# tobwei/APTAI

Hardware: AMD Instinct MI355X
Metric: utterances/sec (10 s @ 16 kHz) train-step (higher is better)
Workload: dtype bf16

## Files before the change

aptai_amd/_lib.py:

```python
from __future__ import annotations

import ctypes
import os
import subprocess
import threading

import torch

_HERE = os.path.dirname(os.path.abspath(__file__))
CSRC = os.path.join(_HERE, "csrc")
LIB_PATH = os.environ.get("APTAI_HIP_LIB") or os.path.join(CSRC, "libaptai_hip.so")

_lib = None
_lock = threading.Lock()

_P, _I64, _I, _F, _U64 = ctypes.c_void_p, ctypes.c_int64, ctypes.c_int, ctypes.c_float, ctypes.c_uint64
ARGTYPES = {
    "aptai_layernorm_fwd": [_P, _P, _P, _P, _P, _P, _I64, _I64, _F, _I, _P],
    "aptai_layernorm_bwd": [_P, _P, _P, _P, _P, _P, _P, _P, _F, _U64, _P, _P, _P, _I64, _I64, _P, _P],
    "aptai_layernorm_bwd_workspace_bytes": [_I64, _I64],
    "aptai_layernorm_bwd_finalize_multi": [_P, _I64, _I64, _P],
    "aptai_layernorm_fwd_f32in": [_P, _P, _P, _P, _P, _I64, _I64, _F, _P],
    "aptai_layernorm_fwd_f32in_split": [_P, _P, _P, _P, _P, _I, _I64, _I64, _F, _P],
    "aptai_attention_fwd": [_P, _P, _P, _P, _P, _I64, _I64, _I64, _I64, _F, _F, _U64, _I, _P],
    "aptai_attention_bwd": [_P, _P, _P, _P, _P, _P, _P, _P, _I64, _I64, _I64, _I64, _F, _F, _U64, _I, _I, _P],
    "aptai_cast_f32_to_bf16": [_P, _P, _I64, _I64, _I64, _P],
    "aptai_conv_weight_to_bf16": [_P, _P, _I64, _I64, _I64, _P],
    "aptai_posconv_weight": [_P, _P, _P, _P, _P, _I64, _I64, _I64, _P],
    "aptai_posconv_pack": [_P, _P, _P, _P, _I64, _I64, _I64, _I64, _I64, _P],
    "aptai_frame_mask_fwd": [_P, _P, _P, _P, _I64, _I64, _I64, _I64, _P],
    "aptai_frame_mask_bwd": [_P, _P, _P, _P, _P, _I64, _I64, _I64, _I64, _P],
    "aptai_frame_mask_bwd_workspace_bytes": [_I64, _I64, _I64],
    "aptai_colsum_bf16": [_P, _I64, _P, _P, _I64, _I64, _I, _P],
    "aptai_colsum_workspace_bytes": [_I64, _I64],
    "aptai_dropout_bf16": [_P, _P, _I64, _F, _U64, _P],
    "aptai_dgelu_bf16": [_P, _P, _P, _I64, _P],
    "aptai_conv0_fwd": [_P, _I64, _I64, _P, _P, _P, _P, _I, _F, _P, _I64, _I64, _I64, _I64, _I64, _P, _P, _P],
    "aptai_conv0_bwd": [_P, _I64, _I64, _P, _P, _P, _P, _I, _F, _P, _I64, _I64, _P, _P, _P, _P, _P, _P, _P],
    "aptai_conv0_bwd_workspace_bytes": [_I64, _I64],
    "aptai_conv0_bwd_data": [_P, _I64, _I64, _P, _P, _P, _P, _I, _F, _P, _I64, _I64, _P, _P, _P, _P],
    "aptai_conv0_bwd_data_workspace_bytes": [_I64, _I64],
    "aptai_conv0_workspace_bytes": [_I64, _I64],
    "aptai_head_act_fwd": [_P, _P, _P, _I64, _F, _F, _U64, _P],
    "aptai_head_act_bwd": [_P, _P, _P, _P, _I64, _F, _F, _U64, _P],
    "aptai_lowpass_fir": [_P, _I64, _I64, _P, _I64, _P, _I64, _I64, _I, _I64, _I64, _I64, _I64, _I64, _P],
    "aptai_aptai_loss_fwd": [_P, _P, _P, _I64, _I64, _P, _I64, _I64, _I64, _I64, _F, _F, _P, _P, _P, _P],
    "aptai_aptai_loss_bwd": [_P, _P, _P, _I64, _I64, _P, _I64, _I64, _I64, _I64, _F, _F, _P, _P, _P, _P, _I64, _P],
    "aptai_aptai_loss_workspace_bytes": [],
# ... 97 lines not shown
```

aptai_amd/csrc/attention.hip:

```cpp
#include "common.h"

namespace {

#ifdef APTAI_STAMPS
__device__ unsigned long long g_attn_stamps[3 * 1024 * 8];
#define ATTN_STAMP(k, slot)                                                                                       \
    do {                                                                                                          \
        if (threadIdx.x == 0) {                                                                                   \
            const int bl = blockIdx.x + gridDim.x * (blockIdx.y + gridDim.y * blockIdx.z);                        \
            if (bl < 1024) g_attn_stamps[((k) * 1024 + bl) * 8 + (slot)] = wall_clock64();                         \
        }                                                                                                         \
    } while (0)
#else
#define ATTN_STAMP(k, slot) do {} while (0)
#endif

constexpr int HD = 64;
constexpr float LOG2E = 1.4426950408889634f;

struct AttnArgs {
    const bf16_t* qkv; long ld;
    const int* lens;
    bf16_t* ctx; long ldo;
    float* lse2;
    float* o32;
    int B, Tp, H, heads;
    float c;
    float scale;
    uint32_t seed0, seed1, thr16; float dscale;
    const uint32_t* salt;
    const bf16_t* dctx;
    float* delta;
    bf16_t* dqkv;
    int skip_pad_q;
    int stagger;
    int xcd_remap;
// ... 54 lines not shown
    const int r31 = lane & 31, h = lane >> 5;
#pragma unroll
    for (int dt = 0; dt < 2; ++dt)
#pragma unroll
        for (int g4 = 0; g4 < 4; ++g4) {
            const int d = dt * 32 + 8 * g4 + 4 * h;
            *(u32x2*)(sw + r31 * OUT_PITCH + d * 2) = (u32x2){pack2bf(acc[dt][4 * g4] * scale, acc[dt][4 * g4 + 1] * scale),
                                                              pack2bf(acc[dt][4 * g4 + 2] * scale, acc[dt][4 * g4 + 3] * scale)};
        }
    __builtin_amdgcn_fence(__ATOMIC_RELEASE, "wavefront");
#pragma unroll
    for (int i = 0; i < 4; ++i) {
        const int idx = i * 64 + lane, r = idx >> 3, ch = idx & 7;
        *(u32x4*)(g_row0 + (long)r * ld + ch * 8) = *(const u32x4*)(sw + r * OUT_PITCH + ch * 16);
    }
    __builtin_amdgcn_fence(__ATOMIC_ACQUIRE, "wavefront");
}

__device__ __forceinline__ bool attn_keep(uint32_t pair, int key, uint32_t s0, uint32_t s1, uint32_t thr16) {
    const uint32_t hsh = rng_hash(pair, s0, s1);
    return ((key & 1) ? (hsh >> 16) : (hsh & 0xffffu)) >= thr16;
}

__device__ __forceinline__ void attn_block(const AttnArgs& a, int& tile, int& hd, int& b) {
    const int nt = gridDim.x, total = nt * gridDim.y * gridDim.z;
    int L = blockIdx.x + nt * (blockIdx.y + gridDim.y * blockIdx.z);
    if (a.xcd_remap && (total & 7) == 0) L = (L & 7) * (total >> 3) + (L >> 3);
    tile = L % nt;
    const int grp = L / nt;
    hd = grp % (int)gridDim.y;
    b = grp / (int)gridDim.y;
}

constexpr int FWD_BUF = 2 * 64 * 128;
constexpr int FWD_SMEM = 2 * FWD_BUF;
constexpr float REF_HEADROOM = 40.0f;
constexpr float REF_SUM_LIMIT = 1.4901161193847656e-08f;

template <bool V> struct Flag { static constexpr bool value = V; };

template <bool DROP>
__global__ __launch_bounds__(256, 3) void attn_fwd_kernel(AttnArgs a) {
    __shared__ __attribute__((aligned(16))) char smem[FWD_SMEM];
    ATTN_STAMP(0, 0);
    if (DROP) apply_salt(a.salt, a.seed0, a.seed1);
    const int tid = threadIdx.x, lane = tid & 63, wave = tid >> 6, h = lane >> 5;
    int tile_x, hd, b;
    attn_block(a, tile_x, hd, b);
    const int q0 = tile_x * 128 + wave * 32;
    int len = a.lens[b];
    len = len < 1 ? 1 : (len > a.Tp ? a.Tp : len);
    const int ntiles = (len + 63) >> 6;
    const long rowbase = (long)b * a.Tp;
    const int q = q0 + (lane & 31);
    const bf16_t* Qg = a.qkv + (rowbase + q) * a.ld + hd * HD;
// ... 153 lines not shown
    if (a.o32) {
#pragma unroll
        for (int dt = 0; dt < 2; ++dt) {
            __syncthreads();
#pragma unroll
            for (int g4 = 0; g4 < 4; ++g4)
                *(f32x4*)(sw + r31 * OUT_PITCH + (8 * g4 + 4 * h) * 4) =
                    (f32x4){oT[dt][4 * g4], oT[dt][4 * g4 + 1], oT[dt][4 * g4 + 2], oT[dt][4 * g4 + 3]};
            __syncthreads();
#pragma unroll
            for (int i = 0; i < 4; ++i) {
                const int idx = i * 64 + lane, r = idx >> 3, ch = idx & 7;
                *(f32x4*)(a.o32 + orow + (long)r * a.ldo + dt * 32 + ch * 4) = *(const f32x4*)(sw + r * OUT_PITCH + ch * 16);
            }
        }
    }
    ATTN_STAMP(0, 3);
#ifdef APTAI_STAMPS
    asm volatile("s_waitcnt vmcnt(0)" ::: "memory");
    ATTN_STAMP(0, 4);
#endif
}

template <bool PRE>
__global__ __launch_bounds__(256, PRE ? DKDV_BLOCKS : 2) void attn_bwd_dkdv_kernel(AttnArgs a) {
    __shared__ __attribute__((aligned(16))) char smem[STAGE_BYTES + 384 + DKDV_KV_BYTES];
    char* sQ = smem;
    char* sD = smem + 32 * 128;
    float* sL = (float*)(smem + STAGE_BYTES);
    char* sKall = smem + STAGE_BYTES + 384;
    char* sVall = sKall + 128 * 128;
    ATTN_STAMP(1, 0);
    if (a.thr16) apply_salt(a.salt, a.seed0, a.seed1);
    const int tid = threadIdx.x, lane = tid & 63, wave = tid >> 6, h = lane >> 5;
    int tile_x, hd, b;
    attn_block(a, tile_x, hd, b);
    const int kb0 = tile_x * 128;
    const int key0 = kb0 + wave * 32;
    int len = a.lens[b];
    len = len < 1 ? 1 : (len > a.Tp ? a.Tp : len);
    const long rowbase = (long)b * a.Tp;
    const int key = key0 + (lane & 31);
    bf16_t* dK0 = a.dqkv + (rowbase + kb0) * a.ld + a.H + hd * HD;
    bf16_t* dV0 = dK0 + a.H;
    if (kb0 >= len) {
        const u32x4 z = {0u, 0u, 0u, 0u};
#pragma unroll
        for (int it = 0; it < 4; ++it) {
            const int cid = it * 256 + tid, row = cid >> 3, ch = cid & 7;
            *(u32x4*)(dK0 + (long)row * a.ld + ch * 8) = z;
            *(u32x4*)(dV0 + (long)row * a.ld + ch * 8) = z;
        }
        return;
    }
    const LaneOffs lo = lane_offs(lane);
    const bf16_t* K0 = a.qkv + (rowbase + kb0) * a.ld + a.H + hd * HD;
    stage_rows128(sKall, K0, a.ld, tid);
    stage_rows128(sVall, K0 + a.H, a.ld, tid);
    f32x16 dKT[2], dVT[2];
    dKT[0] = dKT[1] = dVT[0] = dVT[1] = (f32x16)(0.f);

    const int nq = a.skip_pad_q ? ((len + 31) >> 5) : (a.Tp >> 5);
    const bf16_t* Qb = a.qkv + rowbase * a.ld + hd * HD;
    const bf16_t* Db = a.dctx + rowbase * a.ldo + hd * HD;
    const float* lse = a.lse2 + ((long)b * a.heads + hd) * a.Tp;
    const float* del = a.delta + ((long)b * a.heads + hd) * a.Tp;
    const int srow = tid >> 3, sch = tid & 7;
    const int soff = tile_off(srow, sch);
    const long gq = (long)srow * a.ld + sch * 8, gd = (long)srow * a.ldo + sch * 8;
    u32x4 qreg = *(const u32x4*)(Qb + gq), dreg = *(const u32x4*)(Db + gd);
    const float* stat = (tid < 8 ? lse : del) + (tid & 7) * 4;
    f32x4 sreg = (f32x4)(0.f);
    if (tid < 16) sreg = *(const f32x4*)stat;
    const bool key_ok = key < len;
    const bool wave_boundary = key0 + 32 > len;
    const uint32_t hshift = (key & 1) ? 16u : 0u;
    const float c = a.c;
    const uint32_t pairk = (uint32_t)(key >> 1) * ATTN_K1;
    const uint32_t rowid0 = (uint32_t)((b * a.heads + hd) * a.Tp) + (uint32_t)(tid & 31);
    uint32_t hreg = 0;
    if (a.thr16 && tid >= 32 && tid < 64) hreg = rng_hash(rowid0, a.seed0, a.seed1);
    ATTN_STAMP(1, 1);
    for (int t = 0; t < nq; ++t) {
        __syncthreads();
        *(u32x4*)(sQ + soff) = qreg;
        *(u32x4*)(sD + soff) = dreg;
        if (tid < 16) *(f32x4*)(sL + tid * 4) = PRE ? -sreg : sreg;
        if (a.thr16 && tid >= 32 && tid < 64) ((uint32_t*)sL)[64 + (tid & 31)] = hreg;
        __syncthreads();
        if (t + 1 < nq) {
            qreg = *(const u32x4*)(Qb + (long)(t + 1) * 32 * a.ld + gq);
            dreg = *(const u32x4*)(Db + (long)(t + 1) * 32 * a.ldo + gd);
            if (tid < 16) sreg = *(const f32x4*)(stat + (t + 1) * 32);
            if (a.thr16 && tid >= 32 && tid < 64) hreg = rng_hash(rowid0 + (uint32_t)((t + 1) * 32), a.seed0, a.seed1);
        }
        f32x16 cs = (f32x16)(0.f), cd = (f32x16)(0.f);
        if (PRE) {
#pragma unroll
            for (int g4 = 0; g4 < 4; ++g4) {
                const f32x4 l4 = *(const f32x4*)(sL + 8 * g4 + 4 * h);
                const f32x4 d4 = *(const f32x4*)(sL + 32 + 8 * g4 + 4 * h);
#pragma unroll
                for (int rr = 0; rr < 4; ++rr) { cs[4 * g4 + rr] = l4[rr]; cd[4 * g4 + rr] = d4[rr]; }
            }
        }
        f32x16 s = __builtin_amdgcn_mfma_f32_32x32x16_bf16(rd_row(sQ, lo, 0, 0), rd_row(sKall, lo, wave, 0), cs, 0, 0, 0);
        f32x16 dp = __builtin_amdgcn_mfma_f32_32x32x16_bf16(rd_row(sD, lo, 0, 0), rd_row(sVall, lo, wave, 0), cd, 0, 0, 0);
#pragma unroll
        for (int ds = 1; ds < 4; ++ds) {
            s = __builtin_amdgcn_mfma_f32_32x32x16_bf16(rd_row(sQ, lo, 0, ds), rd_row(sKall, lo, wave, ds), s, 0, 0, 0);
            dp = __builtin_amdgcn_mfma_f32_32x32x16_bf16(rd_row(sD, lo, 0, ds), rd_row(sVall, lo, wave, ds), dp, 0, 0, 0);
        }
        float pd[16], dsv[16];
        if (PRE) {
#pragma unroll
            for (int r = 0; r < 16; ++r) pd[r] = fast_exp2(s[r]);
// ... 26 lines not shown
                    const bool k = ((y >> hshift) & 0xffffu) >= a.thr16;
                    const float p0 = pd[r];
                    if (PRE) dsv[r] = p0 * (k ? dp[r] : nd4[rr]);
                    else dsv[r] = p0 * ((k ? dp[r] : 0.f) - dsv[r]);
                    pd[r] = k ? p0 : 0.f;
                }
            }
        } else {
#pragma unroll
            for (int r = 0; r < 16; ++r) dsv[r] = PRE ? pd[r] * dp[r] : pd[r] * (dp[r] - dsv[r]);
        }
#pragma unroll
        for (int sstep = 0; sstep < 2; ++sstep) {
            const bf16x8 pf = pack8(&pd[8 * sstep]);
            const bf16x8 df = pack8(&dsv[8 * sstep]);
#pragma unroll
            for (int dt = 0; dt < 2; ++dt) {
                dVT[dt] = __builtin_amdgcn_mfma_f32_32x32x16_bf16(rd_tr(sD, lo, sstep, dt), pf, dVT[dt], 0, 0, 0);
                dKT[dt] = __builtin_amdgcn_mfma_f32_32x32x16_bf16(rd_tr(sQ, lo, sstep, dt), df, dKT[dt], 0, 0, 0);
            }
        }
    }
    __syncthreads();
    ATTN_STAMP(1, 2);
    char* sw = smem + wave * (32 * OUT_PITCH);
    store_rows_bf16(sw, dKT, (PRE ? 0.6931471805599453f : a.scale) * a.dscale, dK0 + (long)(wave * 32) * a.ld, a.ld, lane);
    store_rows_bf16(sw, dVT, a.dscale, dV0 + (long)(wave * 32) * a.ld, a.ld, lane);
    ATTN_STAMP(1, 3);
#ifdef APTAI_STAMPS
    asm volatile("s_waitcnt vmcnt(0)" ::: "memory");
    ATTN_STAMP(1, 4);
#endif
}

template <bool PRE>
__global__ __launch_bounds__(256, 3) void attn_bwd_dq_kernel(AttnArgs a) {
    __shared__ __attribute__((aligned(16))) char smem[DQ_STAGE + 512];
    char* sK = smem;
    char* sV = smem + 32 * 128;
    float* sDel = (float*)(smem + DQ_STAGE);
    ATTN_STAMP(2, 0);
    if (a.thr16) apply_salt(a.salt, a.seed0, a.seed1);
    const int tid = threadIdx.x, lane = tid & 63, wave = tid >> 6, h = lane >> 5;
    int tile_x, hd, b;
    attn_block(a, tile_x, hd, b);
    const int qb0 = tile_x * 128;
    const int q = qb0 + wave * 32 + (lane & 31);
    int len = a.lens[b];
    len = len < 1 ? 1 : (len > a.Tp ? a.Tp : len);
    const long rowbase = (long)b * a.Tp;
    const LaneOffs lo = lane_offs(lane);
    bf16x8 qf[4], df[4];
    const bf16_t* Kb = a.qkv + rowbase * a.ld + a.H + hd * HD;
    const bf16_t* Vb = Kb + a.H;
    const int srow = tid >> 3, sch = tid & 7;
    const int soff = tile_off(srow, sch);
    const long gk = (long)srow * a.ld + sch * 8;
    u32x4 kreg = *(const u32x4*)(Kb + gk), vreg = *(const u32x4*)(Vb + gk);
    const bf16_t* Qrows = a.qkv + (rowbase + qb0) * a.ld + hd * HD;
    const bf16_t* Drows = a.dctx + (rowbase + qb0) * a.ldo + hd * HD;
    u32x4 qst[4], dst[4];
#pragma unroll
    for (int it = 0; it < 4; ++it) {
        const int cid = it * 256 + tid, row = cid >> 3, ch = cid & 7;
        qst[it] = *(const u32x4*)(Qrows + (long)row * a.ld + ch * 8);
        dst[it] = *(const u32x4*)(Drows + (long)row * a.ldo + ch * 8);
    }
    const int part = lane & 15, rsub = lane >> 4;
    f32x4 ovv[8];
#pragma unroll
    for (int it = 0; it < 8; ++it) {
        const int row = wave * 32 + it * 4 + rsub;
        const long g = (rowbase + qb0 + row) * a.ldo + hd * HD + part * 4;
        if (a.o32) {
            ovv[it] = *(const f32x4*)(a.o32 + g);
        } else {
            const u32x2 ov = *(const u32x2*)(a.ctx + g);
            ovv[it] = (f32x4){lo_bf(ov[0]), hi_bf(ov[0]), lo_bf(ov[1]), hi_bf(ov[1])};
        }
    }
    const float lse_q = a.lse2[((long)b * a.heads + hd) * a.Tp + q];
    char* sQt = smem;
    char* sDt = smem + 128 * 128;
#pragma unroll
    for (int it = 0; it < 4; ++it) {
        const int cid = it * 256 + tid, row = cid >> 3, ch = cid & 7;
        *(u32x4*)(sQt + tile_off(row, ch)) = qst[it];
        *(u32x4*)(sDt + tile_off(row, ch)) = dst[it];
    }
    ATTN_STAMP(2, 5);
    __syncthreads();
    ATTN_STAMP(2, 6);
#pragma unroll
    for (int ds = 0; ds < 4; ++ds) { qf[ds] = rd_row(sQt, lo, wave, ds); df[ds] = rd_row(sDt, lo, wave, ds); }
#pragma unroll
    for (int it = 0; it < 8; ++it) {
        const int row = wave * 32 + it * 4 + rsub;
        const u32x2 dv = *(const u32x2*)(sDt + tile_off(row, part >> 1) + ((part & 1) << 3));
        float acc = lo_bf(dv[0]) * ovv[it][0];
        acc = fmaf(hi_bf(dv[0]), ovv[it][1], acc);
        acc = fmaf(lo_bf(dv[1]), ovv[it][2], acc);
        acc = fmaf(hi_bf(dv[1]), ovv[it][3], acc);
        acc += __shfl_xor(acc, 8, 64);
        acc += __shfl_xor(acc, 4, 64);
        acc += __shfl_xor(acc, 2, 64);
        acc += __shfl_xor(acc, 1, 64);
        if (part == 0) sDel[row] = acc;
    }
    ATTN_STAMP(2, 7);
    __syncthreads();
    float del_q = sDel[wave * 32 + (lane & 31)];
    __syncthreads();
    del_q *= __frcp_rn(a.dscale);
    if (h == 0) a.delta[((long)b * a.heads + hd) * a.Tp + q] = del_q;
    f32x16 dQT[2];
    dQT[0] = dQT[1] = (f32x16)(0.f);
    const int nk = (len + 31) >> 5;
    uint32_t hbase = 0;
    if (a.thr16) hbase = rng_hash((uint32_t)((b * a.heads + hd) * a.Tp + q), a.seed0, a.seed1) + (uint32_t)(2 * h) * ATTN_K1;
    const float c = a.c;
    const f32x16 cs = (f32x16)(PRE ? -lse_q : 0.f), cd = (f32x16)(PRE ? -del_q : 0.f);
    ATTN_STAMP(2, 1);
    for (int t = 0; t < nk; ++t) {
        __syncthreads();
        *(u32x4*)(sK + soff) = kreg;
        *(u32x4*)(sV + soff) = vreg;
        __syncthreads();
        if (t + 1 < nk) {
            kreg = *(const u32x4*)(Kb + (long)(t + 1) * 32 * a.ld + gk);
            vreg = *(const u32x4*)(Vb + (long)(t + 1) * 32 * a.ld + gk);
        }
        f32x16 sT = __builtin_amdgcn_mfma_f32_32x32x16_bf16(rd_row(sK, lo, 0, 0), qf[0], cs, 0, 0, 0);
        f32x16 dpT = __builtin_amdgcn_mfma_f32_32x32x16_bf16(rd_row(sV, lo, 0, 0), df[0], cd, 0, 0, 0);
#pragma unroll
        for (int ds = 1; ds < 4; ++ds) {
            sT = __builtin_amdgcn_mfma_f32_32x32x16_bf16(rd_row(sK, lo, 0, ds), qf[ds], sT, 0, 0, 0);
            dpT = __builtin_amdgcn_mfma_f32_32x32x16_bf16(rd_row(sV, lo, 0, ds), df[ds], dpT, 0, 0, 0);
        }
        float dsv[16];
        const bool boundary = t * 32 + 32 > len;
#pragma unroll
        for (int r = 0; r < 16; ++r) {
            float p = PRE ? fast_exp2(sT[r]) : fast_exp2(fmaf(sT[r], c, -lse_q));
            if (boundary && (t * 32 + acc_row(r, h) >= len)) p = 0.f;
            dsv[r] = p;
        }
        if (a.thr16) {
            const float dropped = PRE ? -del_q : 0.f;
#pragma unroll
            for (int r = 0; r < 16; r += 2) {
                const uint32_t hsh = attn_mix(hbase + (uint32_t)(t * 16 + acc_row(r, 0) / 2) * ATTN_K1);
                dpT[r] = (hsh & 0xffffu) >= a.thr16 ? dpT[r] : dropped;
                dpT[r + 1] = (hsh >> 16) >= a.thr16 ? dpT[r + 1] : dropped;
            }
        }
#pragma unroll
        for (int r = 0; r < 16; ++r) dsv[r] *= PRE ? dpT[r] : (dpT[r] - del_q);
#pragma unroll
        for (int sstep = 0; sstep < 2; ++sstep) {
            const bf16x8 dsf = pack8(&dsv[8 * sstep]);
#pragma unroll
            for (int dt = 0; dt < 2; ++dt)
                dQT[dt] = __builtin_amdgcn_mfma_f32_32x32x16_bf16(rd_tr(sK, lo, sstep, dt), dsf, dQT[dt], 0, 0, 0);
        }
    }
    __syncthreads();
    ATTN_STAMP(2, 2);
    store_rows_bf16(smem + wave * (32 * OUT_PITCH), dQT, a.scale * a.dscale,
                    a.dqkv + (rowbase + qb0 + wave * 32) * a.ld + hd * HD, a.ld, lane);
    ATTN_STAMP(2, 3);
#ifdef APTAI_STAMPS
    asm volatile("s_waitcnt vmcnt(0)" ::: "memory");
    ATTN_STAMP(2, 4);
#endif
}

__device__ __forceinline__ uint32_t lds_u32x(const char* p) {
    return (uint32_t)(uintptr_t)(__attribute__((address_space(3))) const char*)p;
}

struct AttnXArgs {
    const bf16_t* qkv; long ld;
    const int* lens;
    bf16_t* ctx; long ldo;
    int B, Tp, H, heads, slots;
    float c;
    int xcd_remap;
};

__device__ __forceinline__ void tr_pair_asm(uint32_t a_lo, uint32_t a_hi, short4v& lo, short4v& hi) {
    asm volatile("ds_read_b64_tr_b16 %0, %1" : "=v"(lo) : "v"(a_lo));
    asm volatile("ds_read_b64_tr_b16 %0, %1" : "=v"(hi) : "v"(a_hi));
}
__device__ __forceinline__ bf16x8 tr_join(const short4v lo, const short4v hi) {
    return __builtin_bit_cast(bf16x8, (short8v){lo[0], lo[1], lo[2], lo[3], hi[0], hi[1], hi[2], hi[3]});
}
template <int NPQ>
// ... 178 lines not shown
    }
}

int fill_args(AttnArgs& a, const char* who, const void* qkv, const int32_t* lens, int64_t B, int64_t Tp, int64_t H,
              int64_t heads, float scale, float dropout_p, uint64_t seed, int q_prescaled, const void* stream) {
    APTAI_REQUIRE(qkv && lens, "%s: null pointer", who);
    APTAI_REQUIRE(B > 0 && Tp > 0 && Tp % 128 == 0, "%s: frames per utterance (%ld) must be a positive multiple of 128", who, (long)Tp);
    APTAI_REQUIRE(heads > 0 && H == heads * HD, "%s: head_dim must be 64 (H=%ld heads=%ld)", who, (long)H, (long)heads);
    memset(&a, 0, sizeof(a));
    a.qkv = (const bf16_t*)qkv; a.ld = 3 * H; a.lens = lens; a.ldo = H;
    a.B = (int)B; a.Tp = (int)Tp; a.H = (int)H; a.heads = (int)heads;
    a.scale = scale; a.c = q_prescaled ? 1.0f : scale * LOG2E;
    a.q_prescaled = q_prescaled;
    a.thr16 = drop_thr16(dropout_p); a.dscale = drop_scale(a.thr16);
    a.seed0 = (uint32_t)seed; a.seed1 = (uint32_t)(seed >> 32);
    a.salt = aptai_seed_salt(stream);
    static const int stagger = getenv("APTAI_ATTN_STAGGER") ? atoi(getenv("APTAI_ATTN_STAGGER")) : 0;
    a.stagger = stagger;
    static const int remap = getenv("APTAI_ATTN_XCD_REMAP") ? atoi(getenv("APTAI_ATTN_XCD_REMAP")) : 1;
    a.xcd_remap = remap;
    return APTAI_OK;
}

}

#ifdef APTAI_STAMPS
extern "C" int aptai_debug_read_attn_stamps(void* host_out) {
    return hipMemcpyFromSymbol(host_out, HIP_SYMBOL(g_attn_stamps), sizeof(g_attn_stamps)) == hipSuccess ? 0 : 1;
}
#endif

extern "C" int aptai_attention_fwd(const void* qkv, const int32_t* lens, void* ctx, float* lse2, float* ctx_f32, int64_t B,
                                   int64_t Tp, int64_t H, int64_t heads, float scale, float dropout_p, uint64_t seed,
                                   int q_prescaled, void* stream_) {
    AttnArgs a;
    int rc = fill_args(a, "aptai_attention_fwd", qkv, lens, B, Tp, H, heads, scale, dropout_p, seed, q_prescaled, stream_);
    if (rc) return rc;
    APTAI_REQUIRE(ctx != nullptr, "aptai_attention_fwd: null ctx");
    a.ctx = (bf16_t*)ctx; a.lse2 = lse2; a.o32 = ctx_f32;
    if (a.thr16) {
        APTAI_LAUNCH(attn_fwd_kernel<true>, dim3((unsigned)(Tp / 128), (unsigned)heads, (unsigned)B), dim3(256), 0,
                     (hipStream_t)stream_, a);
    } else {
        APTAI_LAUNCH(attn_fwd_kernel<false>, dim3((unsigned)(Tp / 128), (unsigned)heads, (unsigned)B), dim3(256), 0,
                     (hipStream_t)stream_, a);
    }
    APTAI_CHECK_LAUNCH("attn_fwd_kernel");
    return APTAI_OK;
}

extern "C" int aptai_attention_bwd(const void* qkv, const int32_t* lens, const void* ctx, const float* ctx_f32, const void* dctx,
                                   const float* lse2, float* delta_ws, void* dqkv, int64_t B, int64_t Tp, int64_t H,
                                   int64_t heads, float scale, float dropout_p, uint64_t seed, int dctx_zero_beyond_len,
                                   int q_prescaled, void* stream_) {
    hipStream_t stream = (hipStream_t)stream_;
    AttnArgs a;
    int rc = fill_args(a, "aptai_attention_bwd", qkv, lens, B, Tp, H, heads, scale, dropout_p, seed, q_prescaled, stream_);
    if (rc) return rc;
    APTAI_REQUIRE(ctx && dctx && lse2 && delta_ws && dqkv, "aptai_attention_bwd: null pointer");
    a.ctx = (bf16_t*)ctx; a.dctx = (const bf16_t*)dctx; a.lse2 = (float*)lse2; a.delta = delta_ws; a.o32 = (float*)ctx_f32; a.dqkv = (bf16_t*)dqkv;
    a.skip_pad_q = dctx_zero_beyond_len;
    dim3 grid((unsigned)(Tp / 128), (unsigned)heads, (unsigned)B);
    if (q_prescaled) {
        APTAI_LAUNCH(attn_bwd_dq_kernel<true>, grid, dim3(256), 0, stream, a);
        APTAI_CHECK_LAUNCH("attn_bwd_dq_kernel");
        APTAI_LAUNCH(attn_bwd_dkdv_kernel<true>, grid, dim3(256), 0, stream, a);
    } else {
        APTAI_LAUNCH(attn_bwd_dq_kernel<false>, grid, dim3(256), 0, stream, a);
        APTAI_CHECK_LAUNCH("attn_bwd_dq_kernel");
        APTAI_LAUNCH(attn_bwd_dkdv_kernel<false>, grid, dim3(256), 0, stream, a);
    }
    APTAI_CHECK_LAUNCH("attn_bwd_dkdv_kernel");
    return APTAI_OK;
}

extern "C" int aptai_attention_exact_fwd(const void* qkv_split, int64_t ld, const int32_t* lens, void* ctx_split, int64_t ldo, int64_t B,
                                         int64_t Tp, int64_t H, int64_t heads, int pieces, float scale, void* stream_) {
    APTAI_REQUIRE(qkv_split && lens && ctx_split, "aptai_attention_exact_fwd: null pointer");
    APTAI_REQUIRE(B > 0 && Tp > 0 && Tp % 128 == 0, "aptai_attention_exact_fwd: frames per utterance (%ld) must be a positive multiple of 128", (long)Tp);
    APTAI_REQUIRE(heads > 0 && H == heads * HD, "aptai_attention_exact_fwd: head_dim must be 64 (H=%ld heads=%ld)", (long)H, (long)heads);
    APTAI_REQUIRE(pieces == 3 || pieces == 6, "aptai_attention_exact_fwd: pieces must be 3 (f32x3) or 6 (f32x6)");
    APTAI_REQUIRE(ld >= 3 * pieces * H && ld % 8 == 0 && ldo >= pieces * H && ldo % 8 == 0, "aptai_attention_exact_fwd: row pitches (ld=%ld, ldo=%ld) too small "
                  "for %d slots of H=%ld or not a multiple of 8", (long)ld, (long)ldo, pieces, (long)H);
    APTAI_REQUIRE((uintptr_t)qkv_split % 16 == 0 && (uintptr_t)ctx_split % 16 == 0, "aptai_attention_exact_fwd: operands must be 16-byte aligned");
    AttnXArgs a;
    a.qkv = (const bf16_t*)qkv_split; a.ld = ld; a.lens = lens; a.ctx = (bf16_t*)ctx_split; a.ldo = ldo;
    a.B = (int)B; a.Tp = (int)Tp; a.H = (int)H; a.heads = (int)heads; a.slots = pieces;
    a.c = scale * LOG2E;
    static const int remap = getenv("APTAI_ATTN_XCD_REMAP") ? atoi(getenv("APTAI_ATTN_XCD_REMAP")) : 1;
    a.xcd_remap = remap;
    const dim3 grid((unsigned)(Tp / 128), (unsigned)heads, (unsigned)B);
    if (pieces == 3) {
        constexpr int smem = 2 * 2 * 2 * 64 * 128;
        static const hipError_t attr = hipFuncSetAttribute((const void*)attn_exact_fwd_kernel<2>, hipFuncAttributeMaxDynamicSharedMemorySize, smem);
        APTAI_REQUIRE(attr == hipSuccess, "aptai_attention_exact_fwd: cannot reserve %d bytes of LDS", smem);
// ... 11 lines not shown
```

aptai_amd/ops.py:

```python
from __future__ import annotations

import ctypes
from typing import Optional

import torch

from . import _lib

EPI_BIAS, EPI_GELU, EPI_RESIDUAL, EPI_DROPOUT, EPI_DGELU, EPI_ALPHA, EPI_PRE_DGELU, EPI_MUL_AUX, EPI_RESIDUAL_F32, EPI_SPLIT_OUT, EPI_BIAS_ROW = 1, 2, 4, 8, 16, 32, 64, 128, 256, 512, 1024

c_void_p, c_i64, c_int, c_float, c_u64 = (ctypes.c_void_p, ctypes.c_int64, ctypes.c_int, ctypes.c_float,
                                          ctypes.c_uint64)


class GemmDesc(ctypes.Structure):
    _fields_ = [("A", c_void_p), ("lda", c_i64), ("B", c_void_p), ("ldb", c_i64), ("C", c_void_p), ("ldc", c_i64),
                ("M", c_i64), ("N", c_i64), ("K", c_i64),
                ("a_kmajor", c_int), ("b_kmajor", c_int), ("out_f32", c_int), ("flags", c_int),
                ("bias", c_void_p), ("residual", c_void_p), ("ldr", c_i64), ("out_pre", c_void_p),
                ("aux", c_void_p), ("ldaux", c_i64), ("alpha", c_float), ("dropout_p", c_float), ("seed", c_u64),
                ("split_k", c_int), ("accumulate", c_int), ("workspace", c_void_p), ("workspace_bytes", c_i64),
                ("batch_outer", c_int), ("batch_inner", c_int),
                ("batch_stride_a", c_i64 * 2), ("batch_stride_b", c_i64 * 2), ("batch_stride_c", c_i64 * 2),
                ("batch_stride_bias", c_i64 * 2), ("batch_stride_res", c_i64 * 2), ("batch_stride_aux", c_i64 * 2),
# ... 413 lines not shown

def attention_fwd(qkv, lens_i32, B, Tp, H, heads, *, dropout_p=0.0, seed=0, save_lse=True, q_prescaled=False):
    _dev(qkv, lens_i32)
    ctx = torch.empty((B * Tp, H), device=qkv.device, dtype=torch.bfloat16)
    lse2 = torch.empty((B, heads, Tp), device=qkv.device, dtype=torch.float32) if save_lse else None
    ctx32 = torch.empty((B * Tp, H), device=qkv.device, dtype=torch.float32) if save_lse else None
    _lib.call("aptai_attention_fwd", qkv.data_ptr(), lens_i32.data_ptr(), ctx.data_ptr(), _ptr(lse2), _ptr(ctx32), B, Tp, H,
              heads, (H // heads) ** -0.5, dropout_p, seed, int(q_prescaled), _stream())
    return ctx, (lse2, ctx32) if save_lse else None


def attention_bwd(qkv, lens_i32, ctx, dctx, stats, B, Tp, H, heads, *, dropout_p=0.0, seed=0, dctx_zero_beyond_len=False,
                  q_prescaled=False):
    lse2, ctx32 = stats
    _dev(qkv, lens_i32, ctx, dctx, lse2)
    dqkv = torch.empty_like(qkv)
    delta = torch.empty((B, heads, Tp), device=qkv.device, dtype=torch.float32)
    _lib.call("aptai_attention_bwd", qkv.data_ptr(), lens_i32.data_ptr(), ctx.data_ptr(), _ptr(ctx32), dctx.data_ptr(), lse2.data_ptr(),
              delta.data_ptr(), dqkv.data_ptr(), B, Tp, H, heads, (H // heads) ** -0.5, dropout_p, seed,
              int(dctx_zero_beyond_len), int(q_prescaled), _stream())
    return dqkv


def cast_bf16(src: torch.Tensor, dst: Optional[torch.Tensor] = None, ld_dst: Optional[int] = None) -> torch.Tensor:
    _dev(src, dst)
    src2 = src.reshape(src.shape[0], -1) if src.dim() > 1 else src.reshape(1, -1)
    rows, cols = src2.shape
    if dst is None:
        dst = torch.empty(src.shape, device=src.device, dtype=torch.bfloat16)
    _lib.call("aptai_cast_f32_to_bf16", src2.data_ptr(), dst.data_ptr(), rows, cols, ld_dst if ld_dst else cols, _stream())
    return dst


class CastPlan:

    def __init__(self, jobs):
        self.jobs = list(jobs)
        rows = []
        for src, dst in self.jobs:
            _dev(src, dst)
            n = src.numel()
            if not (src.is_contiguous() and dst.is_contiguous() and src.dtype == torch.float32 and n == dst.numel() and n % 8 == 0
                    and src.data_ptr() % 16 == 0 and dst.data_ptr() % 16 == 0):
                raise _lib.AptaiHipError("CastPlan: jobs must be contiguous, 16-byte aligned fp32 sources of n % 8 == 0 elements")
            kind = {torch.bfloat16: 0, torch.float32: 1}[dst.dtype]
            rows.append([src.data_ptr(), dst.data_ptr(), n, kind])
# ... 439 lines not shown
```

include/aptai_hip.h:

```cpp
#ifndef APTAI_HIP_H
#define APTAI_HIP_H
#include <stdint.h>

#ifdef __cplusplus
extern "C" {
#endif

typedef enum {
    APTAI_OK = 0,
    APTAI_ERR_INVALID = -1,
    APTAI_ERR_LAUNCH = -2,
    APTAI_ERR_NO_DEVICE = -3
} aptai_status;

const char* aptai_last_error(void);
int aptai_version(void);
int aptai_device_check(char* name, int name_len);
int aptai_set_seed_salt(void* stream, const void* device_ptr_2xu32);
int aptai_set_frame_bounds(void* stream, const void* device_ptr_2xi32);

enum {
    APTAI_EPI_BIAS = 1,
    APTAI_EPI_GELU = 2,
    APTAI_EPI_RESIDUAL = 4,
// ... 54 lines not shown
                        void* stream);
int aptai_conv0_fwd_split(const float* audio, int64_t B, int64_t S, const float* weight, const float* bias, const float* gamma,
                          const float* beta, int mode, float eps, void* out_split, int pieces, int64_t T_real, int64_t T_alloc,
                          const float* stats, void* stream);

int aptai_layernorm_fwd(const void* x, const float* gamma, const float* beta, void* y, float* mean, float* rstd,
                        int64_t rows, int64_t cols, float eps, int gelu_after, void* stream);
int aptai_layernorm_fwd_f32in(const float* x, const float* gamma, const float* beta, void* y_bf16, float* y_f32, int64_t rows,
                              int64_t cols, float eps, void* stream);
int aptai_layernorm_fwd_f32in_split(const float* x, const float* gamma, const float* beta, float* y_f32, void* y_split, int pieces,
                                    int64_t rows, int64_t cols, float eps, void* stream);
int aptai_layernorm_bwd(const void* dy, const void* x, const float* mean, const float* rstd, const float* gamma,
                        const void* dres, void* dx, void* dx_drop, float dropout_p, uint64_t seed, float* dgamma,
                        float* dbeta, void* workspace, int64_t rows, int64_t cols, const float* beta_if_gelu_after,
                        void* stream);
int64_t aptai_layernorm_bwd_workspace_bytes(int64_t rows, int64_t cols);
int aptai_layernorm_bwd_finalize_multi(const int64_t* table_dev, int64_t njobs, int64_t max_cols, void* stream);

int aptai_attention_fwd(const void* qkv, const int32_t* lens, void* ctx, float* lse2, float* ctx_f32, int64_t B, int64_t Tp,
                        int64_t H, int64_t heads, float scale, float dropout_p, uint64_t seed, int q_prescaled, void* stream);
int aptai_attention_bwd(const void* qkv, const int32_t* lens, const void* ctx, const float* ctx_f32, const void* dctx,
                        const float* lse2, float* delta_ws, void* dqkv, int64_t B, int64_t Tp, int64_t H, int64_t heads, float scale,
                        float dropout_p, uint64_t seed, int dctx_zero_beyond_len, int q_prescaled, void* stream);

int aptai_cast_f32_to_bf16(const float* src, void* dst, int64_t rows, int64_t cols, int64_t ld_dst, void* stream);
int aptai_cast_multi(const int64_t* table_dev, int64_t njobs, int64_t max_n, void* stream);
int aptai_adam_multi(const int64_t* table_dev, const int64_t* dyn_dev, int64_t njobs, int64_t max_n, float lr, float beta1,
                     float beta2, float eps, float weight_decay, void* stream);
int aptai_conv_weight_to_bf16(const float* src, void* dst, int64_t N, int64_t C, int64_t Kw, void* stream);
int aptai_posconv_weight(const float* v, const float* gain, float* norm_ws, void* w_fwd, void* w_dgrad, int64_t H,
                         int64_t groups, int64_t Kw, void* stream);
int aptai_posconv_weight_bwd(const float* dw_fwd, const float* v, const float* gain, const float* norm, float* dv, float* dgain,
                             float* workspace, int64_t H, int64_t groups, int64_t Kw, void* stream);
int aptai_posconv_gemm(const void* xg, int64_t first_row, const void* w, const float* bias, const void* residual, void* out,
                       void* out_pre, int64_t B, int64_t Tp, int64_t H, int64_t groups, int64_t Kw, int64_t pad, int gelu,
                       void* stream);
int aptai_posconv_wgrad(const void* du_g, const void* x_g, float* dw, int64_t B, int64_t Tp, int64_t H, int64_t groups, int64_t Kw,
                        int64_t pad, void* stream);
int aptai_spec_augment_mask(const int32_t* frame_lens, void* mask_u8, int64_t B, int64_t T, float mask_prob, int64_t mask_length,
                            int64_t min_masks, uint64_t seed, void* stream);
int aptai_posconv_pack(const void* x, const void* u, void* xg, void* rowmajor_out, int64_t B, int64_t Tp, int64_t H,
                       int64_t groups, int64_t pad, void* stream);

int aptai_frame_mask_fwd(void* h, const int32_t* lens, const uint8_t* spec_mask, const float* embed, int64_t B, int64_t Tp,
                         int64_t T, int64_t H, void* stream);
int aptai_frame_mask_bwd(void* dy, const int32_t* lens, const uint8_t* spec_mask, float* dembed, void* workspace, int64_t B,
// ... 101 lines not shown
```

Before: 1715.

## Merge attention backward dQ and dK/dV kernels into one persistent launch

The two attention backward kernels become a single persistent kernel that pulls work items from a global atomic ticket counter. dQ items run first and publish the per-row delta values; dK/dV items spin on a per-(batch, head) counter until every dQ tile of their group has finished. This removes the second launch and the drain between the two kernels so dK/dV work can overlap the tail of the dQ work. In exchange it adds spin-waits, agent-scope atomic loads of the statistics, and a timeout status word that is cleared through a separate host call.

```diff
diff --git a/aptai_amd/_lib.py b/aptai_amd/_lib.py
--- a/aptai_amd/_lib.py
+++ b/aptai_amd/_lib.py
@@ -24,6 +24,7 @@
     "aptai_layernorm_fwd_f32in_split": [_P, _P, _P, _P, _P, _I, _I64, _I64, _F, _P],
     "aptai_attention_fwd": [_P, _P, _P, _P, _P, _I64, _I64, _I64, _I64, _F, _F, _U64, _I, _P],
     "aptai_attention_bwd": [_P, _P, _P, _P, _P, _P, _P, _P, _I64, _I64, _I64, _I64, _F, _F, _U64, _I, _I, _P],
+    "aptai_attention_bwd_status": [_P, _P],
     "aptai_cast_f32_to_bf16": [_P, _P, _I64, _I64, _I64, _P],
     "aptai_conv_weight_to_bf16": [_P, _P, _I64, _I64, _I64, _P],
     "aptai_posconv_weight": [_P, _P, _P, _P, _P, _I64, _I64, _I64, _P],
diff --git a/aptai_amd/csrc/attention.hip b/aptai_amd/csrc/attention.hip
--- a/aptai_amd/csrc/attention.hip
+++ b/aptai_amd/csrc/attention.hip
@@ -1,17 +1,23 @@
 #include "common.h"
+
+#include <mutex>
+#include <vector>
 
 namespace {
 
 #ifdef APTAI_STAMPS
 __device__ unsigned long long g_attn_stamps[3 * 1024 * 8];
+#define ATTN_ITEM_STAMP(k, slot)                                                                                  \
+    do {                                                                                                          \
+        if (threadIdx.x == 0 && stamp_bl < 1024) g_attn_stamps[((k) * 1024 + stamp_bl) * 8 + (slot)] = wall_clock64(); \
+    } while (0)
 #define ATTN_STAMP(k, slot)                                                                                       \
     do {                                                                                                          \
-        if (threadIdx.x == 0) {                                                                                   \
-            const int bl = blockIdx.x + gridDim.x * (blockIdx.y + gridDim.y * blockIdx.z);                        \
-            if (bl < 1024) g_attn_stamps[((k) * 1024 + bl) * 8 + (slot)] = wall_clock64();                         \
-        }                                                                                                         \
+        const int stamp_bl = blockIdx.x + gridDim.x * (blockIdx.y + gridDim.y * blockIdx.z);                      \
+        ATTN_ITEM_STAMP(k, slot);                                                                                 \
     } while (0)
 #else
+#define ATTN_ITEM_STAMP(k, slot) do {} while (0)
 #define ATTN_STAMP(k, slot) do {} while (0)
 #endif
 
@@ -112,15 +118,16 @@
     return ((key & 1) ? (hsh >> 16) : (hsh & 0xffffu)) >= thr16;
 }
 
-__device__ __forceinline__ void attn_block(const AttnArgs& a, int& tile, int& hd, int& b) {
-    const int nt = gridDim.x, total = nt * gridDim.y * gridDim.z;
-    int L = blockIdx.x + nt * (blockIdx.y + gridDim.y * blockIdx.z);
+__device__ __forceinline__ void attn_item(const AttnArgs& a, int L, int& tile, int& hd, int& b) {
+    const int nt = a.Tp >> 7, total = nt * a.heads * a.B;
     if (a.xcd_remap && (total & 7) == 0) L = (L & 7) * (total >> 3) + (L >> 3);
     tile = L % nt;
     const int grp = L / nt;
-    hd = grp % (int)gridDim.y;
-    b = grp / (int)gridDim.y;
-}
+    hd = grp % a.heads;
+    b = grp / a.heads;
+}
+__device__ __forceinline__ int attn_block_index() { return blockIdx.x + gridDim.x * (blockIdx.y + gridDim.y * blockIdx.z); }
+__device__ __forceinline__ void attn_block(const AttnArgs& a, int& tile, int& hd, int& b) { attn_item(a, attn_block_index(), tile, hd, b); }
 
 constexpr int FWD_BUF = 2 * 64 * 128;
 constexpr int FWD_SMEM = 2 * FWD_BUF;
@@ -320,19 +327,41 @@
 #endif
 }
 
+struct BwdSync {
+    unsigned* work = nullptr;
+    unsigned* status = nullptr;
+    unsigned* groups = nullptr;
+};
+constexpr unsigned BWD_SPIN_LIMIT = 1u << 20;
+constexpr unsigned BWD_CONSUMED = 1u << 16;
+typedef __attribute__((address_space(1))) float gfloat;
+
+__device__ __forceinline__ f32x4 ld_sc1_f32x4(const float* p) {
+    gfloat* g = (gfloat*)p;
+    return (f32x4){__hip_atomic_load(g, __ATOMIC_RELAXED, __HIP_MEMORY_SCOPE_AGENT), __hip_atomic_load(g + 1, __ATOMIC_RELAXED, __HIP_MEMORY_SCOPE_AGENT),
+                   __hip_atomic_load(g + 2, __ATOMIC_RELAXED, __HIP_MEMORY_SCOPE_AGENT), __hip_atomic_load(g + 3, __ATOMIC_RELAXED, __HIP_MEMORY_SCOPE_AGENT)};
+}
+__device__ __forceinline__ int item_tid() {
+    int t = threadIdx.x;
+    asm volatile("" : "+v"(t));
+    return t;
+}
+__device__ __forceinline__ void bwd_consumed(unsigned* ctr, int nt) {
+    const unsigned old = __hip_atomic_fetch_add(ctr, BWD_CONSUMED, __ATOMIC_RELAXED, __HIP_MEMORY_SCOPE_AGENT);
+    if ((old >> 16) == (unsigned)nt - 1u) __hip_atomic_store(ctr, 0u, __ATOMIC_RELAXED, __HIP_MEMORY_SCOPE_AGENT);
+}
+
+constexpr int DKDV_SMEM = STAGE_BYTES + 384 + DKDV_KV_BYTES;
 template <bool PRE>
-__global__ __launch_bounds__(256, PRE ? DKDV_BLOCKS : 2) void attn_bwd_dkdv_kernel(AttnArgs a) {
-    __shared__ __attribute__((aligned(16))) char smem[STAGE_BYTES + 384 + DKDV_KV_BYTES];
+__device__ __forceinline__ void bwd_dkdv_item(const AttnArgs& a, char* smem, const int tile_x, const int hd, const int b, const BwdSync& sy,
+                                              const int stamp_bl) {
     char* sQ = smem;
     char* sD = smem + 32 * 128;
     float* sL = (float*)(smem + STAGE_BYTES);
     char* sKall = smem + STAGE_BYTES + 384;
     char* sVall = sKall + 128 * 128;
-    ATTN_STAMP(1, 0);
-    if (a.thr16) apply_salt(a.salt, a.seed0, a.seed1);
-    const int tid = threadIdx.x, lane = tid & 63, wave = tid >> 6, h = lane >> 5;
-    int tile_x, hd, b;
-    attn_block(a, tile_x, hd, b);
+    ATTN_ITEM_STAMP(1, 0);
+    const int tid = item_tid(), lane = tid & 63, wave = tid >> 6, h = lane >> 5;
     const int kb0 = tile_x * 128;
     const int key0 = kb0 + wave * 32;
     int len = a.lens[b];
@@ -341,7 +370,9 @@
     const int key = key0 + (lane & 31);
     bf16_t* dK0 = a.dqkv + (rowbase + kb0) * a.ld + a.H + hd * HD;
     bf16_t* dV0 = dK0 + a.H;
+    unsigned* ctr = sy.groups ? sy.groups + (b * a.heads + hd) : nullptr;
     if (kb0 >= len) {
+        if (ctr && tid == 0) bwd_consumed(ctr, a.Tp >> 7);
         const u32x4 z = {0u, 0u, 0u, 0u};
 #pragma unroll
         for (int it = 0; it < 4; ++it) {
@@ -350,6 +381,18 @@
             *(u32x4*)(dV0 + (long)row * a.ld + ch * 8) = z;
         }
         return;
+    }
+    if (ctr) {
+        if (tid == 0) {
+            const unsigned nt = (unsigned)(a.Tp >> 7);
+            for (unsigned spins = 0; (__hip_atomic_load(ctr, __ATOMIC_RELAXED, __HIP_MEMORY_SCOPE_AGENT) & 0xffffu) < nt;) {
+                if (++spins > BWD_SPIN_LIMIT) { atomicExch(sy.status, 1u); break; }
+                __builtin_amdgcn_s_sleep(2);
+            }
+            bwd_consumed(ctr, (int)nt);
+        }
+        __builtin_amdgcn_fence(__ATOMIC_ACQUIRE, "wavefront");
+        __syncthreads();
     }
     const LaneOffs lo = lane_offs(lane);
     const bf16_t* K0 = a.qkv + (rowbase + kb0) * a.ld + a.H + hd * HD;
@@ -369,7 +412,7 @@
     u32x4 qreg = *(const u32x4*)(Qb + gq), dreg = *(const u32x4*)(Db + gd);
     const float* stat = (tid < 8 ? lse : del) + (tid & 7) * 4;
     f32x4 sreg = (f32x4)(0.f);
-    if (tid < 16) sreg = *(const f32x4*)stat;
+    if (tid < 16) sreg = ld_sc1_f32x4(stat);
     const bool key_ok = key < len;
     const bool wave_boundary = key0 + 32 > len;
     const uint32_t hshift = (key & 1) ? 16u : 0u;
@@ -378,7 +421,7 @@
     const uint32_t rowid0 = (uint32_t)((b * a.heads + hd) * a.Tp) + (uint32_t)(tid & 31);
     uint32_t hreg = 0;
     if (a.thr16 && tid >= 32 && tid < 64) hreg = rng_hash(rowid0, a.seed0, a.seed1);
-    ATTN_STAMP(1, 1);
+    ATTN_ITEM_STAMP(1, 1);
     for (int t = 0; t < nq; ++t) {
         __syncthreads();
         *(u32x4*)(sQ + soff) = qreg;
@@ -389,7 +432,7 @@
         if (t + 1 < nq) {
             qreg = *(const u32x4*)(Qb + (long)(t + 1) * 32 * a.ld + gq);
             dreg = *(const u32x4*)(Db + (long)(t + 1) * 32 * a.ldo + gd);
-            if (tid < 16) sreg = *(const f32x4*)(stat + (t + 1) * 32);
+            if (tid < 16) sreg = ld_sc1_f32x4(stat + (t + 1) * 32);
             if (a.thr16 && tid >= 32 && tid < 64) hreg = rng_hash(rowid0 + (uint32_t)((t + 1) * 32), a.seed0, a.seed1);
         }
         f32x16 cs = (f32x16)(0.f), cd = (f32x16)(0.f);
@@ -462,28 +505,35 @@
         }
     }
     __syncthreads();
-    ATTN_STAMP(1, 2);
+    ATTN_ITEM_STAMP(1, 2);
     char* sw = smem + wave * (32 * OUT_PITCH);
     store_rows_bf16(sw, dKT, (PRE ? 0.6931471805599453f : a.scale) * a.dscale, dK0 + (long)(wave * 32) * a.ld, a.ld, lane);
     store_rows_bf16(sw, dVT, a.dscale, dV0 + (long)(wave * 32) * a.ld, a.ld, lane);
-    ATTN_STAMP(1, 3);
+    ATTN_ITEM_STAMP(1, 3);
 #ifdef APTAI_STAMPS
     asm volatile("s_waitcnt vmcnt(0)" ::: "memory");
-    ATTN_STAMP(1, 4);
+    ATTN_ITEM_STAMP(1, 4);
 #endif
 }
 
 template <bool PRE>
-__global__ __launch_bounds__(256, 3) void attn_bwd_dq_kernel(AttnArgs a) {
-    __shared__ __attribute__((aligned(16))) char smem[DQ_STAGE + 512];
+__global__ __launch_bounds__(256, PRE ? DKDV_BLOCKS : 2) void attn_bwd_dkdv_kernel(AttnArgs a) {
+    __shared__ __attribute__((aligned(16))) char smem[DKDV_SMEM];
+    if (a.thr16) apply_salt(a.salt, a.seed0, a.seed1);
+    int tile_x, hd, b;
+    attn_block(a, tile_x, hd, b);
+    bwd_dkdv_item<PRE>(a, smem, tile_x, hd, b, BwdSync{}, attn_block_index());
+}
+
+constexpr int DQ_SMEM = DQ_STAGE + 512;
+template <bool PRE>
+__device__ __forceinline__ void bwd_dq_item(const AttnArgs& a, char* smem, const int tile_x, const int hd, const int b, const BwdSync& sy,
+                                            const int stamp_bl) {
     char* sK = smem;
     char* sV = smem + 32 * 128;
     float* sDel = (float*)(smem + DQ_STAGE);
-    ATTN_STAMP(2, 0);
-    if (a.thr16) apply_salt(a.salt, a.seed0, a.seed1);
-    const int tid = threadIdx.x, lane = tid & 63, wave = tid >> 6, h = lane >> 5;
-    int tile_x, hd, b;
-    attn_block(a, tile_x, hd, b);
+    ATTN_ITEM_STAMP(2, 0);
+    const int tid = item_tid(), lane = tid & 63, wave = tid >> 6, h = lane >> 5;
     const int qb0 = tile_x * 128;
     const int q = qb0 + wave * 32 + (lane & 31);
     int len = a.lens[b];
@@ -528,9 +578,9 @@
         *(u32x4*)(sQt + tile_off(row, ch)) = qst[it];
         *(u32x4*)(sDt + tile_off(row, ch)) = dst[it];
     }
-    ATTN_STAMP(2, 5);
+    ATTN_ITEM_STAMP(2, 5);
     __syncthreads();
-    ATTN_STAMP(2, 6);
+    ATTN_ITEM_STAMP(2, 6);
 #pragma unroll
     for (int ds = 0; ds < 4; ++ds) { qf[ds] = rd_row(sQt, lo, wave, ds); df[ds] = rd_row(sDt, lo, wave, ds); }
 #pragma unroll
@@ -547,12 +597,17 @@
         acc += __shfl_xor(acc, 1, 64);
         if (part == 0) sDel[row] = acc;
     }
-    ATTN_STAMP(2, 7);
+    ATTN_ITEM_STAMP(2, 7);
     __syncthreads();
     float del_q = sDel[wave * 32 + (lane & 31)];
     __syncthreads();
     del_q *= __frcp_rn(a.dscale);
-    if (h == 0) a.delta[((long)b * a.heads + hd) * a.Tp + q] = del_q;
+    if (h == 0) __hip_atomic_store((gfloat*)(a.delta + ((long)b * a.heads + hd) * a.Tp + q), del_q, __ATOMIC_RELAXED, __HIP_MEMORY_SCOPE_AGENT);
+    if (sy.groups) {
+        asm volatile("s_waitcnt vmcnt(0)" ::: "memory");
+        __syncthreads();
+        if (tid == 0) __hip_atomic_fetch_add(sy.groups + (b * a.heads + hd), 1u, __ATOMIC_RELAXED, __HIP_MEMORY_SCOPE_AGENT);
+    }
     f32x16 dQT[2];
     dQT[0] = dQT[1] = (f32x16)(0.f);
     const int nk = (len + 31) >> 5;
@@ -560,7 +615,7 @@
     if (a.thr16) hbase = rng_hash((uint32_t)((b * a.heads + hd) * a.Tp + q), a.seed0, a.seed1) + (uint32_t)(2 * h) * ATTN_K1;
     const float c = a.c;
     const f32x16 cs = (f32x16)(PRE ? -lse_q : 0.f), cd = (f32x16)(PRE ? -del_q : 0.f);
-    ATTN_STAMP(2, 1);
+    ATTN_ITEM_STAMP(2, 1);
     for (int t = 0; t < nk; ++t) {
         __syncthreads();
         *(u32x4*)(sK + soff) = kreg;
@@ -605,14 +660,52 @@
         }
     }
     __syncthreads();
-    ATTN_STAMP(2, 2);
+    ATTN_ITEM_STAMP(2, 2);
     store_rows_bf16(smem + wave * (32 * OUT_PITCH), dQT, a.scale * a.dscale,
                     a.dqkv + (rowbase + qb0 + wave * 32) * a.ld + hd * HD, a.ld, lane);
-    ATTN_STAMP(2, 3);
+    ATTN_ITEM_STAMP(2, 3);
 #ifdef APTAI_STAMPS
     asm volatile("s_waitcnt vmcnt(0)" ::: "memory");
-    ATTN_STAMP(2, 4);
+    ATTN_ITEM_STAMP(2, 4);
 #endif
+}
+
+template <bool PRE>
+__global__ __launch_bounds__(256, 3) void attn_bwd_dq_kernel(AttnArgs a) {
+    __shared__ __attribute__((aligned(16))) char smem[DQ_SMEM];
+    if (a.thr16) apply_salt(a.salt, a.seed0, a.seed1);
+    int tile_x, hd, b;
+    attn_block(a, tile_x, hd, b);
+    bwd_dq_item<PRE>(a, smem, tile_x, hd, b, BwdSync{}, attn_block_index());
+}
+
+template <bool PRE>
+__global__ __launch_bounds__(256, PRE ? DKDV_BLOCKS : 2) void attn_bwd_kernel(AttnArgs a, BwdSync sy) {
+    __shared__ __attribute__((aligned(16))) char smem[DKDV_SMEM > DQ_SMEM ? DKDV_SMEM : DQ_SMEM];
+    __shared__ int s_item;
+    if (a.thr16) apply_salt(a.salt, a.seed0, a.seed1);
+    const int n = (a.Tp >> 7) * a.heads * a.B;
+    const unsigned last_ticket = (unsigned)(2 * n) - 1u;
+    int item = blockIdx.x;
+    for (;;) {
+        int tile_x, hd, b;
+        if (item < n) {
+            attn_item(a, item, tile_x, hd, b);
+            bwd_dq_item<PRE>(a, smem, tile_x, hd, b, sy, item);
+        } else {
+            attn_item(a, item - n, tile_x, hd, b);
+            bwd_dkdv_item<PRE>(a, smem, tile_x, hd, b, sy, item - n);
+        }
+        __syncthreads();
+        if (threadIdx.x == 0) {
+            const unsigned t = __hip_atomic_fetch_add(sy.work, 1u, __ATOMIC_RELAXED, __HIP_MEMORY_SCOPE_AGENT);
+            if (t == last_ticket) __hip_atomic_store(sy.work, 0u, __ATOMIC_RELAXED, __HIP_MEMORY_SCOPE_AGENT);
+            s_item = (int)(t + gridDim.x);
+        }
+        __syncthreads();
+        item = s_item;
+        if (item >= 2 * n) break;
+    }
 }
 
 __device__ __forceinline__ uint32_t lds_u32x(const char* p) {
@@ -837,6 +930,40 @@
     return APTAI_OK;
 }
 
+constexpr int BWD_SYNC_SLOTS = 16, BWD_SYNC_HDR = 64, BWD_SYNC_GROUPS = 4096, BWD_SYNC_WORDS = BWD_SYNC_HDR + BWD_SYNC_GROUPS;
+constexpr int BWD_SYNC_DEVICES = 64;
+__device__ unsigned g_attn_bwd_sync[BWD_SYNC_SLOTS * BWD_SYNC_WORDS];
+
+int bwd_sync_slot(hipStream_t stream, int64_t groups, unsigned** slot, int* cus, bool create = true) {
+    static std::mutex mu;
+    static std::vector<hipStream_t> keys[BWD_SYNC_DEVICES];
+    static unsigned* base[BWD_SYNC_DEVICES] = {};
+    static int ncu[BWD_SYNC_DEVICES] = {};
+    *slot = nullptr;
+    if (groups > BWD_SYNC_GROUPS) return APTAI_OK;
+    int dev = 0;
+    APTAI_REQUIRE(hipGetDevice(&dev) == hipSuccess && dev >= 0 && dev < BWD_SYNC_DEVICES, "aptai_attention_bwd: no usable device");
+    std::lock_guard<std::mutex> lock(mu);
+    if (base[dev] == nullptr) {
+        void* p = nullptr;
+        APTAI_REQUIRE(hipGetSymbolAddress(&p, HIP_SYMBOL(g_attn_bwd_sync)) == hipSuccess && p != nullptr,
+                      "aptai_attention_bwd: cannot locate the counter slots");
+        APTAI_REQUIRE(hipDeviceGetAttribute(&ncu[dev], hipDeviceAttributeMultiprocessorCount, dev) == hipSuccess && ncu[dev] > 0,
+                      "aptai_attention_bwd: cannot read the CU count");
+        base[dev] = (unsigned*)p;
+    }
+    if (cus) *cus = ncu[dev];
+    std::vector<hipStream_t>& k = keys[dev];
+    size_t i = 0;
+    while (i < k.size() && k[i] != stream) ++i;
+    if (i == k.size()) {
+        if (!create || i >= (size_t)BWD_SYNC_SLOTS) return APTAI_OK;
+        k.push_back(stream);
+    }
+    *slot = base[dev] + i * BWD_SYNC_WORDS;
+    return APTAI_OK;
+}
+
 }
 
 #ifdef APTAI_STAMPS
@@ -875,6 +1002,25 @@
     APTAI_REQUIRE(ctx && dctx && lse2 && delta_ws && dqkv, "aptai_attention_bwd: null pointer");
     a.ctx = (bf16_t*)ctx; a.dctx = (const bf16_t*)dctx; a.lse2 = (float*)lse2; a.delta = delta_ws; a.o32 = (float*)ctx_f32; a.dqkv = (bf16_t*)dqkv;
     a.skip_pad_q = dctx_zero_beyond_len;
+    static const int one_launch = getenv("APTAI_ATTN_BWD_ONE_LAUNCH") ? atoi(getenv("APTAI_ATTN_BWD_ONE_LAUNCH")) : 1;
+    unsigned* sync = nullptr;
+    int cus = 0;
+    if (one_launch) {
+        rc = bwd_sync_slot(stream, B * heads, &sync, &cus);
+        if (rc) return rc;
+    }
+    if (sync) {
+        const long items = 2 * (Tp / 128) * heads * B;
+        long grid = (long)(q_prescaled ? DKDV_BLOCKS : 2) * cus;
+        if (grid > items) grid = items;
+        APTAI_REQUIRE(items + grid < (1L << 31), "aptai_attention_bwd: too many work items (%ld)", items);
+        BwdSync sy;
+        sy.work = sync; sy.status = sync + 1; sy.groups = sync + BWD_SYNC_HDR;
+        if (q_prescaled) APTAI_LAUNCH(attn_bwd_kernel<true>, dim3((unsigned)grid), dim3(256), 0, stream, a, sy);
+        else APTAI_LAUNCH(attn_bwd_kernel<false>, dim3((unsigned)grid), dim3(256), 0, stream, a, sy);
+        APTAI_CHECK_LAUNCH("attn_bwd_kernel");
+        return APTAI_OK;
+    }
     dim3 grid((unsigned)(Tp / 128), (unsigned)heads, (unsigned)B);
     if (q_prescaled) {
         APTAI_LAUNCH(attn_bwd_dq_kernel<true>, grid, dim3(256), 0, stream, a);
@@ -886,6 +1032,22 @@
         APTAI_LAUNCH(attn_bwd_dkdv_kernel<false>, grid, dim3(256), 0, stream, a);
     }
     APTAI_CHECK_LAUNCH("attn_bwd_dkdv_kernel");
+    return APTAI_OK;
+}
+
+extern "C" int aptai_attention_bwd_status(void* stream, int* status_out) {
+    APTAI_REQUIRE(status_out != nullptr, "aptai_attention_bwd_status: null pointer");
+    *status_out = 0;
+    unsigned* sync = nullptr;
+    int rc = bwd_sync_slot((hipStream_t)stream, 0, &sync, nullptr, false);
+    if (rc || sync == nullptr) return rc;
+    unsigned v = 0;
+    if (hipMemcpyAsync(&v, sync + 1, 4, hipMemcpyDeviceToHost, (hipStream_t)stream) != hipSuccess ||
+        hipStreamSynchronize((hipStream_t)stream) != hipSuccess)
+        APTAI_FAIL(APTAI_ERR_LAUNCH, "aptai_attention_bwd_status: reading the status word failed");
+    if (v != 0 && hipMemsetAsync(sync, 0, BWD_SYNC_WORDS * 4, (hipStream_t)stream) != hipSuccess)
+        APTAI_FAIL(APTAI_ERR_LAUNCH, "aptai_attention_bwd_status: clearing the slot failed");
+    *status_out = (int)v;
     return APTAI_OK;
 }
 
diff --git a/aptai_amd/ops.py b/aptai_amd/ops.py
--- a/aptai_amd/ops.py
+++ b/aptai_amd/ops.py
@@ -459,6 +459,13 @@
     return dqkv
 
 
+def attention_bwd_check() -> None:
+    out = ctypes.c_int(0)
+    _lib.check(_lib.lib().aptai_attention_bwd_status(c_void_p(_stream()), ctypes.byref(out)), "aptai_attention_bwd_status")
+    if out.value != 0:
+        raise _lib.AptaiHipError("aptai_attention_bwd: a dK/dV item's wait for the delta values of its dQ items timed out")
+
+
 def cast_bf16(src: torch.Tensor, dst: Optional[torch.Tensor] = None, ld_dst: Optional[int] = None) -> torch.Tensor:
     _dev(src, dst)
     src2 = src.reshape(src.shape[0], -1) if src.dim() > 1 else src.reshape(1, -1)
diff --git a/include/aptai_hip.h b/include/aptai_hip.h
--- a/include/aptai_hip.h
+++ b/include/aptai_hip.h
@@ -100,6 +100,7 @@
 int aptai_attention_bwd(const void* qkv, const int32_t* lens, const void* ctx, const float* ctx_f32, const void* dctx,
                         const float* lse2, float* delta_ws, void* dqkv, int64_t B, int64_t Tp, int64_t H, int64_t heads, float scale,
                         float dropout_p, uint64_t seed, int dctx_zero_beyond_len, int q_prescaled, void* stream);
+int aptai_attention_bwd_status(void* stream, int* status_out);
 
 int aptai_cast_f32_to_bf16(const float* src, void* dst, int64_t rows, int64_t cols, int64_t ld_dst, void* stream);
 int aptai_cast_multi(const int64_t* table_dev, int64_t njobs, int64_t max_n, void* stream);
```

After: 1667 (median of 2 runs). 0.972x the previous value.
